# GAP-LAB-CUHK-SZ/REC-MV

Hardware: AMD Instinct MI355X
Metric: optimiser iters/sec, female-3-casual-like 512x512 (synthetic frames) (higher is better)
Workload: dtype f32

## Files before the change

rec-mv_amd/csrc/common.h:

```cpp
#pragma once
#include <hip/hip_runtime.h>
#include <stdint.h>
#include <stdio.h>
#include <string.h>
#include "../../include/recmv_hip.h"

namespace recmv {

void set_error(const char* fmt, ...);

inline int check_launch(const char* what) {
  hipError_t e = hipGetLastError();
  if (e != hipSuccess) {
    set_error("%s: %s", what, hipGetErrorString(e));
    return RECMV_ERR_HIP;
  }
  return RECMV_OK;
}

#define RECMV_HIP_TRY(expr)                                              \
  do {                                                                   \
    hipError_t e__ = (expr);                                             \
    if (e__ != hipSuccess) {                                             \
      ::recmv::set_error("%s: %s", #expr, hipGetErrorString(e__));       \
      return RECMV_ERR_HIP;                                              \
    }                                                                    \
  } while (0)

#define RECMV_REQUIRE(cond, ...)                                         \
  do {                                                                   \
    if (!(cond)) {                                                       \
      ::recmv::set_error(__VA_ARGS__);                                   \
      return RECMV_ERR_ARG;                                              \
    }                                                                    \
  } while (0)

constexpr int kWave = 64;
constexpr int kNumCU = 256;
constexpr int kNumXCD = 8;

inline int64_t ceil_div(int64_t a, int64_t b) { return (a + b - 1) / b; }

inline int stream_grid(int64_t work_items, int block) {
  int64_t g = ceil_div(work_items, block);
  const int64_t cap = (int64_t)kNumCU * 8;
  if (g > cap) g = cap;
  if (g < 1) g = 1;
  return (int)g;
}

}
```

rec-mv_amd/csrc/gemm_f32.hip:

```cpp
#include <mutex>
#include <unordered_map>
#include <type_traits>
#include <vector>
#include "common.h"
#ifdef RECMV_LIBM_SOFTPLUS
#define RECMV_EXPF(x) expf(x)
#define RECMV_LOG1PF(t) log1pf(t)
#else
#define RECMV_EXPF(x) __expf(x)
#define RECMV_LOG1PF(t) __logf(1.f + (t))
#endif

#include <algorithm>

namespace recmv {
namespace {

typedef float f32x16 __attribute__((ext_vector_type(16)));
typedef float f32x2 __attribute__((ext_vector_type(2)));
typedef __bf16 bf16x2 __attribute__((ext_vector_type(2)));
typedef __bf16 bf16x8 __attribute__((ext_vector_type(8)));
typedef unsigned int u32x4 __attribute__((ext_vector_type(4)));

struct Pieces {
  bf16x8 h, m, l;
};
__device__ __forceinline__ unsigned pack_bf16(float a, float b) {
#ifdef RECMV_SPLIT_INT
  unsigned ua = __float_as_uint(a), ub = __float_as_uint(b);
  ua += 0x7fffu + ((ua >> 16) & 1u);
  ub += 0x7fffu + ((ub >> 16) & 1u);
  return (ua >> 16) | (ub & 0xffff0000u);
#else
  const f32x2 v = {a, b};
  return __builtin_bit_cast(unsigned, __builtin_convertvector(v, bf16x2));
#endif
}
__device__ __forceinline__ void split2(float x0, float x1, unsigned& h, unsigned& m, unsigned& l) {
  h = pack_bf16(x0, x1);
  const f32x2 r = {x0 - __uint_as_float(h << 16), x1 - __uint_as_float(h & 0xffff0000u)};
  m = pack_bf16(r.x, r.y);
  const f32x2 q = {r.x - __uint_as_float(m << 16), r.y - __uint_as_float(m & 0xffff0000u)};
  l = pack_bf16(q.x, q.y);
}
__device__ __forceinline__ Pieces split8(float4 a, float4 b) {
  unsigned h[4], m[4], l[4];
  split2(a.x, a.y, h[0], m[0], l[0]);
  split2(a.z, a.w, h[1], m[1], l[1]);
  split2(b.x, b.y, h[2], m[2], l[2]);
  split2(b.z, b.w, h[3], m[3], l[3]);
  Pieces p;
  p.h = __builtin_bit_cast(bf16x8, (u32x4){h[0], h[1], h[2], h[3]});
  p.m = __builtin_bit_cast(bf16x8, (u32x4){m[0], m[1], m[2], m[3]});
  p.l = __builtin_bit_cast(bf16x8, (u32x4){l[0], l[1], l[2], l[3]});
  return p;
}

constexpr int BM = 128, BN = 128, BK = 32;
constexpr int kBlk = 256;
constexpr int LDK = BK + 4;
constexpr int LDM = BM + 4;

__device__ __forceinline__ int64_t xcd_remap(int64_t b, int64_t nb) {
  const int64_t per = nb / kNumXCD;
  if (b >= per * kNumXCD) return b;
  return (b % kNumXCD) * per + b / kNumXCD;
}

template <int ACT>
__device__ __forceinline__ float apply_act(float z, float p, float inv_p) {
  if (ACT == RECMV_ACT_RELU) return z > 0.f ? z : 0.f;
  if (ACT == RECMV_ACT_SOFTPLUS) {
    const float zb = z * p;
    const float t = RECMV_EXPF(-fabsf(zb));
    const float series = t * (1.f - t * (0.5f - t * (0.33333334f - 0.25f * t)));
    const float l = t < 0.015625f ? series : RECMV_LOG1PF(t);
    const float y = (fmaxf(zb, 0.f) + l) * inv_p;
    return zb > 20.f ? z : y;
  }
  if (ACT == RECMV_ACT_TANH) return tanhf(z);
  return z;
}

__device__ __forceinline__ float dact_y(float y, int act, float p) {
  switch (act) {
    case RECMV_ACT_RELU: return y > 0.f ? 1.f : 0.f;
    case RECMV_ACT_SOFTPLUS: {
      const float t = p * y;
      const float series = t * (1.f - t * (0.5f - t * (0.16666667f - 0.041666668f * t)));
      return t < 0.015625f ? series : 1.f - RECMV_EXPF(-t);
    }
    case RECMV_ACT_TANH: return 1.f - y * y;
    default: return 1.f;
  }
}

struct AMul {
  const float* Y;
  int64_t ldy;
  int act;
  float param, y_scale, a_scale;
  const float* B2;
  const float* bias2;
  int split;
};

__device__ __forceinline__ float4 amul4(float4 a, float4 y, const AMul& m) {
  a.x *= dact_y(y.x * m.y_scale, m.act, m.param) * m.a_scale;
  a.y *= dact_y(y.y * m.y_scale, m.act, m.param) * m.a_scale;
  a.z *= dact_y(y.z * m.y_scale, m.act, m.param) * m.a_scale;
  a.w *= dact_y(y.w * m.y_scale, m.act, m.param) * m.a_scale;
  return a;
}

__device__ __forceinline__ float4 load4_guard(const float* __restrict__ p, int64_t limit, bool vec_ok) {
  float4 v = make_float4(0.f, 0.f, 0.f, 0.f);
  if (limit >= 4 && vec_ok) {
    v = *reinterpret_cast<const float4*>(p);
  } else {
    if (limit > 0) v.x = p[0];
    if (limit > 1) v.y = p[1];
    if (limit > 2) v.z = p[2];
    if (limit > 3) v.w = p[3];
  }
  return v;
}

__device__ __forceinline__ float4 emul4(float4 v, const AMul& m, int gm, int gn, int N) {
  const float* y = m.Y + (int64_t)gm * m.ldy + gn;
  float4 yv = make_float4(0.f, 0.f, 0.f, 0.f);
  if (gn + 4 <= N && (m.ldy & 3) == 0 && (reinterpret_cast<uintptr_t>(m.Y) & 15) == 0) {
    yv = *reinterpret_cast<const float4*>(y);
  } else {
    yv.x = y[0];
    if (gn + 1 < N) yv.y = y[1];
    if (gn + 2 < N) yv.z = y[2];
    if (gn + 3 < N) yv.w = y[3];
  }
  v.x *= dact_y(yv.x * m.y_scale, m.act, m.param) * m.a_scale;
  v.y *= dact_y(yv.y * m.y_scale, m.act, m.param) * m.a_scale;
  v.z *= dact_y(yv.z * m.y_scale, m.act, m.param) * m.a_scale;
  v.w *= dact_y(yv.w * m.y_scale, m.act, m.param) * m.a_scale;
  return v;
}

template <int TBM, int TBN, int ACT>
__device__ __forceinline__ void nt_epilogue_rows(const float* __restrict__ Cs, const float* __restrict__ bias,
                                                 float* __restrict__ C, int64_t ldc, int M, int N, int m0, int n0,
                                                 float act_param, float out_scale, bool c_vec, const AMul& em) {
  constexpr int LDC = TBN + 4;
  constexpr int C4 = TBN / 4;
  constexpr int ROWS_PER_PASS = kBlk / C4;
  const int tid = threadIdx.x;
  const int c4 = tid % C4, r0 = tid / C4;
  const int gn = n0 + c4 * 4;
  if (gn >= N) return;
  const float inv_p = act_param != 0.f ? 1.f / act_param : 0.f;
  float4 bv = make_float4(0.f, 0.f, 0.f, 0.f);
  if (bias) {
    bv.x = bias[gn];
    if (gn + 1 < N) bv.y = bias[gn + 1];
    if (gn + 2 < N) bv.z = bias[gn + 2];
    if (gn + 3 < N) bv.w = bias[gn + 3];
  }
  const bool full4 = c_vec && gn + 4 <= N;
#pragma unroll 2
  for (int row = r0; row < TBM; row += ROWS_PER_PASS) {
    const int gm = m0 + row;
    if (gm >= M) break;
    float4 v = *reinterpret_cast<const float4*>(Cs + row * LDC + c4 * 4);
    v.x = apply_act<ACT>(v.x + bv.x, act_param, inv_p) * out_scale;
    v.y = apply_act<ACT>(v.y + bv.y, act_param, inv_p) * out_scale;
    v.z = apply_act<ACT>(v.z + bv.z, act_param, inv_p) * out_scale;
    v.w = apply_act<ACT>(v.w + bv.w, act_param, inv_p) * out_scale;
    if (em.Y) v = emul4(v, em, gm, gn, N);
    float* dst = C + (int64_t)gm * ldc + gn;
    if (full4) {
      *reinterpret_cast<float4*>(dst) = v;
    } else {
      dst[0] = v.x;
      if (gn + 1 < N) dst[1] = v.y;
      if (gn + 2 < N) dst[2] = v.z;
      if (gn + 3 < N) dst[3] = v.w;
    }
  }
}

template <int T, int ACT>
__device__ __forceinline__ void nt_epilogue(const float* __restrict__ Cs, const float* __restrict__ bias,
                                            float* __restrict__ C, int64_t ldc, int M, int N, int m0, int n0,
                                            float act_param, float out_scale, bool c_vec, const AMul& em) {
  nt_epilogue_rows<64 * T, 64 * T, ACT>(Cs, bias, C, ldc, M, N, m0, n0, act_param, out_scale, c_vec, em);
}

template <int T, bool FAST, bool AMUL, bool BF3>
__global__ __launch_bounds__(kBlk) void gemm_nt_kernel(const float* __restrict__ A, int64_t lda,
                                                       const float* __restrict__ B, int64_t ldb,
                                                       const float* __restrict__ bias, float* __restrict__ C,
                                                       int64_t ldc, int M, int N, int K, int act,
                                                       float act_param, float out_scale, int nbm, int nbn,
                                                       bool a_vec, bool b_vec, bool c_vec, AMul am) {
  constexpr int TBM = 64 * T, TBN = 64 * T;
  constexpr int WT = 32 * T;
  constexpr int NLD = TBM * 8 / kBlk;
  extern __shared__ __attribute__((aligned(16))) float smem[];
  float* As = smem;
  float* Bs = smem + 2 * TBM * LDK;
  const int tid = threadIdx.x, lane = tid & 63, wave = tid >> 6;
  const int wm = wave >> 1, wn = wave & 1;
  const int64_t logical = xcd_remap(blockIdx.x, (int64_t)nbm * nbn);
  const int tile_m = (int)(logical / nbn), tile_n = (int)(logical % nbn);
  const int m0 = tile_m * TBM, n0 = tile_n * TBN;
  if (am.B2 && m0 >= am.split) {
    B = am.B2;
    bias = am.bias2;
  }

  f32x16 acc[T][T];
#pragma unroll
  for (int a = 0; a < T; ++a)
#pragma unroll
    for (int b = 0; b < T; ++b)
#pragma unroll
      for (int r = 0; r < 16; ++r) acc[a][b][r] = 0.f;

// ... 895 lines not shown

  f32x16 acc[2][2];
#pragma unroll
  for (int a = 0; a < 2; ++a)
#pragma unroll
    for (int b = 0; b < 2; ++b)
#pragma unroll
      for (int r = 0; r < 16; ++r) acc[a][b][r] = 0.f;

  float4 ra[NLD], rb[NLD];
  const bool whole_mn = m0 + BM <= M && n0 + BN <= N;
  auto gload = [&](int64_t k0) {
    const bool whole = whole_mn && k0 + BKT <= kend;
#pragma unroll
    for (int r = 0; r < NLD; ++r) {
      const int idx = tid + kBlk * r;
      const int krow = idx >> 5, c4 = idx & 31;
      const int64_t k = k0 + krow;
      const int cm = m0 + c4 * 4, cn = n0 + c4 * 4;
      if (whole) {
        ra[r] = *reinterpret_cast<const float4*>(A + k * lda + cm);
        rb[r] = *reinterpret_cast<const float4*>(B + k * ldb + cn);
      } else {
        const bool kin = k < kend, ain = kin && cm < M, bin = kin && cn < N;
        const int64_t kc = kin ? k : kend - 1;
        float4 a = *reinterpret_cast<const float4*>(A + kc * lda + (cm < M ? cm : (M - 1) & ~3));
        float4 b = *reinterpret_cast<const float4*>(B + kc * ldb + (cn < N ? cn : (N - 1) & ~3));
        ra[r] = make_float4(ain ? a.x : 0.f, ain ? a.y : 0.f, ain ? a.z : 0.f, ain ? a.w : 0.f);
        rb[r] = make_float4(bin ? b.x : 0.f, bin ? b.y : 0.f, bin ? b.z : 0.f, bin ? b.w : 0.f);
      }
    }
  };
  auto lstore = [&]() {
#pragma unroll
    for (int r = 0; r < NLD; ++r) {
      const int idx = tid + kBlk * r;
      const int krow = idx >> 5, c4 = idx & 31;
      *reinterpret_cast<float4*>(As + krow * LDM + c4 * 4) = ra[r];
      *reinterpret_cast<float4*>(Bs + krow * LDM + c4 * 4) = rb[r];
    }
  };

  const int nk = (int)((kend - kbeg + BKT - 1) / BKT);
  if (nk > 0) {
    gload(kbeg);
    lstore();
  }
  __syncthreads();
  const int acol = wm * 64 + (lane & 31), bcol = wn * 64 + (lane & 31), kh = lane >> 5;
  const float* as = As + kh * LDM + acol;
  const float* bs = Bs + kh * LDM + bcol;
  for (int kt = 0; kt < nk; ++kt) {
    if (kt + 1 < nk) gload(kbeg + (int64_t)(kt + 1) * BKT);
#pragma unroll
    for (int k2 = 0; k2 < BKT / 2; ++k2) {
      const float a0 = as[k2 * 2 * LDM], a1 = as[k2 * 2 * LDM + 32];
      const float b0 = bs[k2 * 2 * LDM], b1 = bs[k2 * 2 * LDM + 32];
      acc[0][0] = __builtin_amdgcn_mfma_f32_32x32x2f32(a0, b0, acc[0][0], 0, 0, 0);
      acc[0][1] = __builtin_amdgcn_mfma_f32_32x32x2f32(a0, b1, acc[0][1], 0, 0, 0);
      acc[1][0] = __builtin_amdgcn_mfma_f32_32x32x2f32(a1, b0, acc[1][0], 0, 0, 0);
      acc[1][1] = __builtin_amdgcn_mfma_f32_32x32x2f32(a1, b1, acc[1][1], 0, 0, 0);
    }
    __syncthreads();
    if (kt + 1 < nk) lstore();
    __syncthreads();
  }

  float* Ps = P + (int64_t)split * M * N;
#pragma unroll
  for (int ni = 0; ni < 2; ++ni) {
    const int gn = n0 + wn * 64 + ni * 32 + (lane & 31);
    if (gn >= N) continue;
#pragma unroll
    for (int mi = 0; mi < 2; ++mi) {
#pragma unroll
      for (int r = 0; r < 16; ++r) {
        const int gm = m0 + wm * 64 + mi * 32 + (r & 3) + 8 * (r >> 2) + 4 * (lane >> 5);
        if (gm < M) Ps[(int64_t)gm * N + gn] = acc[mi][ni][r];
      }
    }
  }
}

__global__ __launch_bounds__(kBlk) void splitk_reduce_kernel(const float* __restrict__ P, float* __restrict__ C,
                                                             int64_t ldc, int M, int N, int splits) {
  const int64_t total = (int64_t)M * N;
  for (int64_t i = (int64_t)blockIdx.x * kBlk + threadIdx.x; i < total; i += (int64_t)gridDim.x * kBlk) {
    float s = 0.f;
    for (int sp = 0; sp < splits; ++sp) s += P[(int64_t)sp * total + i];
    C[(i / N) * ldc + (i % N)] = s;
  }
}

__global__ __launch_bounds__(kBlk) void splitk_reduce4_kernel(const float4* __restrict__ P, float* __restrict__ C,
                                                              int64_t ldc, int M, int N, int splits) {
  const int64_t total4 = (int64_t)M * N / 4;
  for (int64_t i = (int64_t)blockIdx.x * kBlk + threadIdx.x; i < total4; i += (int64_t)gridDim.x * kBlk) {
    float4 s = make_float4(0.f, 0.f, 0.f, 0.f);
    int sp = 0;
    for (; sp + 8 <= splits; sp += 8) {
      float4 v[8];
#pragma unroll
      for (int u = 0; u < 8; ++u) v[u] = P[(int64_t)(sp + u) * total4 + i];
#pragma unroll
      for (int u = 0; u < 8; ++u) {
        s.x += v[u].x;
        s.y += v[u].y;
        s.z += v[u].z;
        s.w += v[u].w;
      }
    }
    for (; sp < splits; ++sp) {
      const float4 v = P[(int64_t)sp * total4 + i];
      s.x += v.x;
      s.y += v.y;
      s.z += v.z;
      s.w += v.w;
    }
    const int64_t e = i * 4;
    *reinterpret_cast<float4*>(C + (e / N) * ldc + (e % N)) = s;
  }
}

struct PeWeights {
  float w[32];
};
__global__ __launch_bounds__(kBlk) void posenc_kernel(const float* __restrict__ x, int64_t ldx,
                                                      float* __restrict__ out, int64_t ldo, int64_t ldo_fill,
                                                      int64_t P, int L, PeWeights w, float out_scale) {
  const int nf = 1 + 2 * L;
  const int64_t total = P * nf;
  for (int64_t e = (int64_t)blockIdx.x * kBlk + threadIdx.x; e < total; e += (int64_t)gridDim.x * kBlk) {
    const int64_t p = e / nf;
    const int f = (int)(e % nf);
    const float x0 = x[p * ldx], x1 = x[p * ldx + 1], x2 = x[p * ldx + 2];
    float* o = out + p * ldo + 3 * f;
    if (f == 0) {
      o[0] = x0 * out_scale;
      o[1] = x1 * out_scale;
      o[2] = x2 * out_scale;
      for (int64_t c = 3 * nf; c < ldo_fill; ++c) out[p * ldo + c] = 0.f;
    } else {
      const int band = (f - 1) >> 1;
      const float freq = (float)(1 << band);
      const float wt = w.w[f - 1];
      float v0, v1, v2;
      if ((f - 1) & 1) {
        v0 = cosf(x0 * freq); v1 = cosf(x1 * freq); v2 = cosf(x2 * freq);
      } else {
        v0 = sinf(x0 * freq); v1 = sinf(x1 * freq); v2 = sinf(x2 * freq);
      }
      o[0] = wt * v0 * out_scale;
      o[1] = wt * v1 * out_scale;
      o[2] = wt * v2 * out_scale;
    }
  }
}

struct LaunchRec {
  hipEvent_t a, b;
  int variant;
  double flops, bytes;
};
struct Profiler {
  bool on = false;
  double min_flops = 0.0;
  double untimed[14][2] = {};
  std::vector<LaunchRec> recs;
  std::vector<hipEvent_t> pool;
  double large[14][3] = {};
  double timed_bytes[14] = {};
  double busy_union_s = 0.0, busy_span_s = 0.0;
  std::mutex mu;
  hipEvent_t get() {
    std::lock_guard<std::mutex> lk(mu);
    if (!pool.empty()) {
      hipEvent_t e = pool.back();
      pool.pop_back();
      return e;
    }
    hipEvent_t e;
    if (hipEventCreate(&e) != hipSuccess) return nullptr;
    return e;
  }
};
Profiler g_prof;

struct ScopedLaunchTimer {
  LaunchRec r;
  hipStream_t s;
  bool active;
  ScopedLaunchTimer(int variant, double M, double N, double K, hipStream_t stream) : s(stream), active(g_prof.on) {
    if (!active) return;
    const double flops = 2.0 * M * N * K;
    r.bytes = 4.0 * (M * K + N * K + M * N);
    if (flops < g_prof.min_flops) {
      std::lock_guard<std::mutex> lk(g_prof.mu);
      g_prof.untimed[variant][0] += 1.0;
      g_prof.untimed[variant][1] += flops;
      active = false;
      return;
    }
    r.variant = variant;
// ... 212 lines not shown
  }
  std::lock_guard<std::mutex> lock(g_b3_mu);
  g_b3[B] = B3Entry{(const char*)planes, N, K, ldb, Kp};
  return RECMV_OK;
}

extern "C" int recmv_b3_forget(const float* B) {
  std::lock_guard<std::mutex> lock(g_b3_mu);
  g_b3.erase(B);
  return RECMV_OK;
}

extern "C" int recmv_gemm_nt(const float* A, int64_t lda, const float* B, int64_t ldb, const float* bias,
                             float* C, int64_t ldc, int64_t M, int64_t N, int64_t K, int act,
                             float act_param, float out_scale, void* stream) {
  RECMV_REQUIRE(M >= 0 && N >= 0 && K >= 0, "gemm_nt: negative size");
  if (M == 0 || N == 0) return RECMV_OK;
  RECMV_REQUIRE(A && B && C, "gemm_nt: NULL pointer");
  RECMV_REQUIRE(lda >= K && ldb >= K && ldc >= N, "gemm_nt: leading dimension too small");
  RECMV_REQUIRE(M < (1ll << 31) - BM && N < (1ll << 31) - BN && K < (1ll << 31) - BK, "gemm_nt: size overflow");
  RECMV_REQUIRE(act >= RECMV_ACT_NONE && act <= RECMV_ACT_TANH, "gemm_nt: unknown activation %d", act);
  AMul am = {nullptr, 0, RECMV_ACT_NONE, 0.f, 1.f, 1.f};
  return dispatch_nt<false>(A, lda, B, ldb, bias, C, ldc, M, N, K, act, act_param, out_scale, am, (hipStream_t)stream);
}

extern "C" int recmv_gemm_nt_actgrad(const float* G, int64_t ldg, const float* Y, int64_t ldy, const float* B,
                                     int64_t ldb, float* C, int64_t ldc, int64_t M, int64_t N, int64_t K, int act,
                                     float act_param, float y_scale, float g_scale, void* stream) {
  RECMV_REQUIRE(M >= 0 && N >= 0 && K >= 0, "gemm_nt_actgrad: negative size");
  if (M == 0 || N == 0) return RECMV_OK;
  RECMV_REQUIRE(G && Y && B && C, "gemm_nt_actgrad: NULL pointer");
  RECMV_REQUIRE((ldg >= K || ldg == 0) && ldy >= K && ldb >= K && ldc >= N,
                "gemm_nt_actgrad: leading dimension too small");
  RECMV_REQUIRE(M < (1ll << 31) - BM && N < (1ll << 31) - BN && K < (1ll << 31) - BK, "gemm_nt_actgrad: size overflow");
  RECMV_REQUIRE(act >= RECMV_ACT_NONE && act <= RECMV_ACT_TANH, "gemm_nt_actgrad: unknown activation %d", act);
  AMul am = {Y, ldy, act, act_param, y_scale, g_scale};
  return dispatch_nt<true>(G, ldg, B, ldb, nullptr, C, ldc, M, N, K, RECMV_ACT_NONE, 0.f, 1.f, am, (hipStream_t)stream);
}

extern "C" int recmv_gemm_nt_mulgrad(const float* A, int64_t lda, const float* B, int64_t ldb, float* C, int64_t ldc,
                                     int64_t M, int64_t N, int64_t K, const float* Y, int64_t ldy, int act,
                                     float act_param, float y_scale, float scale, void* stream) {
  RECMV_REQUIRE(M >= 0 && N >= 0 && K >= 0, "gemm_nt_mulgrad: negative size");
  if (M == 0 || N == 0) return RECMV_OK;
  RECMV_REQUIRE(A && B && C && Y, "gemm_nt_mulgrad: NULL pointer");
  RECMV_REQUIRE(lda >= K && ldb >= K && ldc >= N && ldy >= N, "gemm_nt_mulgrad: leading dimension too small");
  RECMV_REQUIRE(M < (1ll << 31) - BM && N < (1ll << 31) - BN && K < (1ll << 31) - BK, "gemm_nt_mulgrad: size overflow");
  RECMV_REQUIRE(act >= RECMV_ACT_NONE && act <= RECMV_ACT_TANH, "gemm_nt_mulgrad: unknown activation %d", act);
  AMul em = {Y, ldy, act, act_param, y_scale, scale};
  return dispatch_nt<false>(A, lda, B, ldb, nullptr, C, ldc, M, N, K, RECMV_ACT_NONE, 0.f, 1.f, em, (hipStream_t)stream);
}

extern "C" int recmv_gemm_nt_seg(const float* A, int64_t lda, const float* B, int64_t ldb, const float* bias,
                                 const float* B2, const float* bias2, int64_t split_row, float* C, int64_t ldc, int64_t M,
                                 int64_t N, int64_t K, int act, float act_param, float out_scale, void* stream) {
  RECMV_REQUIRE(M >= 0 && N >= 0 && K >= 0, "gemm_nt_seg: negative size");
  if (M == 0 || N == 0) return RECMV_OK;
  RECMV_REQUIRE(A && B && C, "gemm_nt_seg: NULL pointer");
  RECMV_REQUIRE(lda >= K && ldb >= K && ldc >= N, "gemm_nt_seg: leading dimension too small");
  RECMV_REQUIRE(M < (1ll << 31) - BM && N < (1ll << 31) - BN && K < (1ll << 31) - BK, "gemm_nt_seg: size overflow");
  RECMV_REQUIRE(act >= RECMV_ACT_NONE && act <= RECMV_ACT_TANH, "gemm_nt_seg: unknown activation %d", act);
  RECMV_REQUIRE(!B2 || (split_row >= 0 && split_row % BM == 0), "gemm_nt_seg: split_row must be a multiple of %d", BM);
  RECMV_REQUIRE(!B2 || !bias == !bias2, "gemm_nt_seg: both nets with or both without a bias");
  AMul am = {nullptr, 0, RECMV_ACT_NONE, 0.f, 1.f, 1.f, B2, bias2, (int)(split_row < M ? split_row : M)};
  return dispatch_nt<false>(A, lda, B, ldb, bias, C, ldc, M, N, K, act, act_param, out_scale, am, (hipStream_t)stream);
}

extern "C" int recmv_gemm_nt_mulgrad_seg(const float* A, int64_t lda, const float* B, const float* B2, int64_t split_row,
                                         int64_t ldb, float* C, int64_t ldc, int64_t M, int64_t N, int64_t K, const float* Y,
                                         int64_t ldy, int act, float act_param, float y_scale, float scale, void* stream) {
  RECMV_REQUIRE(M >= 0 && N >= 0 && K >= 0, "gemm_nt_mulgrad_seg: negative size");
  if (M == 0 || N == 0) return RECMV_OK;
  RECMV_REQUIRE(A && B && C && Y, "gemm_nt_mulgrad_seg: NULL pointer");
  RECMV_REQUIRE(lda >= K && ldb >= K && ldc >= N && ldy >= N, "gemm_nt_mulgrad_seg: leading dimension too small");
  RECMV_REQUIRE(M < (1ll << 31) - BM && N < (1ll << 31) - BN && K < (1ll << 31) - BK, "gemm_nt_mulgrad_seg: size overflow");
  RECMV_REQUIRE(act >= RECMV_ACT_NONE && act <= RECMV_ACT_TANH, "gemm_nt_mulgrad_seg: unknown activation %d", act);
  RECMV_REQUIRE(!B2 || (split_row >= 0 && split_row % BM == 0), "gemm_nt_mulgrad_seg: split_row must be a multiple of %d", BM);
  AMul em = {Y, ldy, act, act_param, y_scale, scale, B2, nullptr, (int)(split_row < M ? split_row : M)};
  return dispatch_nt<false>(A, lda, B, ldb, nullptr, C, ldc, M, N, K, RECMV_ACT_NONE, 0.f, 1.f, em, (hipStream_t)stream);
}

extern "C" int64_t recmv_gemm_tn_workspace_bytes(int64_t M, int64_t N, int64_t K) {
  if (M <= 0 || N <= 0 || K <= 0) return 0;
  return (int64_t)tn_splits(M, N, K) * M * N * 4;
}

extern "C" int recmv_gemm_tn(const float* A, int64_t lda, const float* B, int64_t ldb, float* C, int64_t ldc,
                             int64_t M, int64_t N, int64_t K, void* workspace, int64_t workspace_bytes,
                             void* stream) {
  RECMV_REQUIRE(M >= 0 && N >= 0 && K >= 0, "gemm_tn: negative size");
  if (M == 0 || N == 0) return RECMV_OK;
  RECMV_REQUIRE(A && B && C, "gemm_tn: NULL pointer");
  RECMV_REQUIRE(lda >= M && ldb >= N && ldc >= N, "gemm_tn: leading dimension too small");
  RECMV_REQUIRE(M < (1 << 20) && N < (1 << 20), "gemm_tn: output too large");
  hipStream_t s = (hipStream_t)stream;
  if (K == 0) {
    for (int64_t m = 0; m < M; ++m) RECMV_HIP_TRY(hipMemsetAsync(C + m * ldc, 0, N * 4, s));
    return RECMV_OK;
  }
  const int splits = tn_splits(M, N, K);
  const int64_t need = (int64_t)splits * M * N * 4;
  if (!workspace || workspace_bytes < need) {
    set_error("gemm_tn: workspace %lld < %lld bytes", (long long)workspace_bytes, (long long)need);
    return RECMV_ERR_WORKSPACE;
  }
  static bool attr_set = false;
  if (!attr_set) {
    RECMV_HIP_TRY(hipFuncSetAttribute((const void*)gemm_tn_kernel<false>, hipFuncAttributeMaxDynamicSharedMemorySize,
                                      kTnLds));
    RECMV_HIP_TRY(hipFuncSetAttribute((const void*)gemm_tn_kernel<true>, hipFuncAttributeMaxDynamicSharedMemorySize,
                                      kTnLds));
    attr_set = true;
  }
  const int nbm = (int)ceil_div(M, BM), nbn = (int)ceil_div(N, BN);
  int64_t kchunk = ceil_div(ceil_div(K, splits), BK) * BK;
  const bool a_vec = aligned16(A) && lda % 4 == 0, b_vec = aligned16(B) && ldb % 4 == 0;
  int rc;
  {
  ScopedLaunchTimer timer(8, (double)M, (double)N, (double)K, s);
  const bool bf3_tn = g_gemm_mode == 1 && (g_b3_families & 4);
  if (!bf3_tn && tn_occ() && a_vec && b_vec && lda >= ((M + 3) & ~3ll) && ldb >= ((N + 3) & ~3ll) && M >= 4 && N >= 4) {
    kchunk = ceil_div(ceil_div(K, splits), 16) * 16;
    hipLaunchKernelGGL(gemm_tn_occ_kernel<16>, dim3((unsigned)(nbm * nbn * splits)), dim3(kBlk), 2 * 16 * LDM * 4, s, A, lda,
                       B, ldb, (float*)workspace, (int)M, (int)N, K, nbm, nbn, kchunk);
  } else if (bf3_tn)
    hipLaunchKernelGGL(gemm_tn_kernel<true>, dim3((unsigned)(nbm * nbn * splits)), dim3(kBlk), kTnLds, s, A, lda, B,
                       ldb, (float*)workspace, (int)M, (int)N, K, nbm, nbn, kchunk, a_vec, b_vec);
  else
    hipLaunchKernelGGL(gemm_tn_kernel<false>, dim3((unsigned)(nbm * nbn * splits)), dim3(kBlk), kTnLds, s, A, lda, B,
                       ldb, (float*)workspace, (int)M, (int)N, K, nbm, nbn, kchunk, a_vec, b_vec);
  rc = check_launch("gemm_tn");
  }
  if (rc) return rc;
  if (N % 4 == 0 && ldc % 4 == 0 && aligned16(C) && aligned16(workspace))
    hipLaunchKernelGGL(splitk_reduce4_kernel, dim3(stream_grid(M * N / 4, kBlk)), dim3(kBlk), 0, s,
                       (const float4*)workspace, C, ldc, (int)M, (int)N, splits);
  else
    hipLaunchKernelGGL(splitk_reduce_kernel, dim3(stream_grid(M * N, kBlk)), dim3(kBlk), 0, s,
                       (const float*)workspace, C, ldc, (int)M, (int)N, splits);
  return check_launch("gemm_tn/reduce");
}

extern "C" int recmv_posenc_forward(const float* x, int64_t ldx, float* out, int64_t ldo, int64_t ldo_fill,
                                    int64_t P, int L, const float* weights_host, float out_scale,
                                    void* stream) {
  RECMV_REQUIRE(P >= 0 && L >= 0 && L <= 16, "posenc: bad size (P=%lld, L=%d)", (long long)P, L);
  if (P == 0) return RECMV_OK;
  RECMV_REQUIRE(x && out, "posenc: NULL pointer");
  RECMV_REQUIRE(ldx >= 3 && ldo >= 3 + 6 * L && ldo_fill <= ldo, "posenc: leading dimension too small");
  hipStream_t s = (hipStream_t)stream;
  PeWeights hw;
  for (int i = 0; i < 32; ++i) hw.w[i] = (weights_host && i < 2 * L) ? weights_host[i] : 1.f;
  hipLaunchKernelGGL(posenc_kernel, dim3(stream_grid(P * (1 + 2 * L), kBlk)), dim3(kBlk), 0, s, x, ldx, out, ldo,
                     ldo_fill, P, L, hw, out_scale);
  return check_launch("posenc");
}

extern "C" int recmv_profile_begin(double min_flops) {
  g_prof.recs.clear();
  for (auto& u : g_prof.untimed) u[0] = u[1] = 0.0;
  g_prof.min_flops = min_flops;
  g_prof.on = true;
  return RECMV_OK;
}

extern "C" int recmv_profile_bytes(double* out, int n_variants) {
  RECMV_REQUIRE(out && n_variants >= 9, "profile_bytes: need room for 9 variants");
  for (int i = 0; i < n_variants; ++i) out[i] = 0.0;
  auto slot = [&](int v) { return v < n_variants ? v : (v == 11 ? 7 : (v == 12 ? 2 : (v == 13 ? 6 : 3))); };
  for (int v = 0; v < 14; ++v) out[slot(v)] += g_prof.timed_bytes[v];
  return RECMV_OK;
}

extern "C" int recmv_profile_large(double* out, int n_variants) {
  RECMV_REQUIRE(out && n_variants >= 9, "profile_large: need room for 9 variants");
  for (int i = 0; i < 3 * n_variants; ++i) out[i] = 0.0;
  auto slot = [&](int v) { return v < n_variants ? v : (v == 11 ? 7 : (v == 12 ? 2 : (v == 13 ? 6 : 3))); };
  for (int v = 0; v < 14; ++v)
    for (int q = 0; q < 3; ++q) out[3 * slot(v) + q] += g_prof.large[v][q];
  return RECMV_OK;
}

extern "C" int recmv_profile_busy(double* out2) {
  RECMV_REQUIRE(out2, "profile_busy: NULL");
  out2[0] = g_prof.busy_union_s;
  out2[1] = g_prof.busy_span_s;
  return RECMV_OK;
}

extern "C" int recmv_profile_end(double* out, int n_variants) {
  g_prof.on = false;
  RECMV_REQUIRE(out && n_variants >= 9, "profile_end: need room for 9 variants");
  for (int i = 0; i < 5 * n_variants; ++i) out[i] = 0.0;
  auto slot = [&](int v) { return v < n_variants ? v : (v == 11 ? 7 : (v == 12 ? 2 : (v == 13 ? 6 : 3))); };
  for (int v = 0; v < 14; ++v) {
    out[5 * slot(v) + 3] += g_prof.untimed[v][0];
    out[5 * slot(v) + 4] += g_prof.untimed[v][1];
  }
  std::vector<std::pair<double, double>> iv;
  iv.reserve(g_prof.recs.size());
  hipEvent_t origin = g_prof.recs.empty() ? nullptr : g_prof.recs.front().a;
  for (auto& b : g_prof.timed_bytes) b = 0.0;
  for (auto& l : g_prof.large) l[0] = l[1] = l[2] = 0.0;
  for (auto& r : g_prof.recs) {
    g_prof.timed_bytes[r.variant] += r.bytes;
    RECMV_HIP_TRY(hipEventSynchronize(r.b));
    float ms = 0.f;
    RECMV_HIP_TRY(hipEventElapsedTime(&ms, r.a, r.b));
    if (r.flops >= 4.0e9) {
      g_prof.large[r.variant][0] += 1.0;
      g_prof.large[r.variant][1] += (double)ms * 1e-3;
      g_prof.large[r.variant][2] += r.flops;
    }
    out[5 * slot(r.variant) + 0] += 1.0;
    out[5 * slot(r.variant) + 1] += (double)ms * 1e-3;
    out[5 * slot(r.variant) + 2] += r.flops;
    float t0 = 0.f;
    if (r.a != origin && hipEventElapsedTime(&t0, origin, r.a) != hipSuccess) t0 = -1.f;
    if (t0 >= 0.f) iv.emplace_back((double)t0 * 1e-3, (double)(t0 + ms) * 1e-3);
  }
  for (auto& r : g_prof.recs) {
    g_prof.pool.push_back(r.a);
    g_prof.pool.push_back(r.b);
  }
  g_prof.recs.clear();
// ... 20 lines not shown
```

rec-mv_amd/csrc/linear_bwd.hip:

```cpp
#include "common.h"

namespace recmv {
namespace {

constexpr int kBlk = 256;
constexpr int kColTile = 64;
constexpr int kMaxChunks = 96;

__global__ __launch_bounds__(kBlk) void colsum_partial_kernel(const float* __restrict__ g, int64_t ld, int64_t rows,
                                                              int cols, int64_t rows_per_chunk,
                                                              float* __restrict__ partial) {
  __shared__ float sh[kBlk / kColTile][kColTile];
  const int ctile = blockIdx.x, chunk = blockIdx.y;
  const int lane = threadIdx.x % kColTile, rgrp = threadIdx.x / kColTile;
  const int c = ctile * kColTile + lane;
  const int64_t r0 = (int64_t)chunk * rows_per_chunk;
  int64_t r1 = r0 + rows_per_chunk;
  if (r1 > rows) r1 = rows;
  float s = 0.f;
  if (c < cols)
    for (int64_t r = r0 + rgrp; r < r1; r += kBlk / kColTile) s += g[r * ld + c];
  sh[rgrp][lane] = s;
  __syncthreads();
  if (rgrp == 0 && c < cols) {
    float t = 0.f;
#pragma unroll
    for (int q = 0; q < kBlk / kColTile; ++q) t += sh[q][lane];
    partial[(int64_t)chunk * cols + c] = t;
  }
}

__device__ __forceinline__ float dact_y(float y, int act, float p) {
  switch (act) {
    case RECMV_ACT_RELU: return y > 0.f ? 1.f : 0.f;
    case RECMV_ACT_SOFTPLUS: return -expm1f(-p * y);
    case RECMV_ACT_TANH: return 1.f - y * y;
    default: return 1.f;
  }
}

template <int VEC>
__global__ __launch_bounds__(kBlk) void act_grad_colsum_kernel(const float* __restrict__ gy, int64_t ldg,
                                                               const float* __restrict__ y, int64_t ldy,
                                                               float* __restrict__ gz, int64_t ldz, int64_t rows,
                                                               int cols, int64_t rows_per_chunk, int act, float p,
                                                               float* __restrict__ partial) {
  constexpr int CT = kColTile / VEC;
  constexpr int RG = kBlk / CT;
  __shared__ float sh[RG][kColTile];
  const int ctile = blockIdx.x, chunk = blockIdx.y;
  const int cl = threadIdx.x % CT, rgrp = threadIdx.x / CT;
  const int c = ctile * kColTile + cl * VEC;
  const int64_t r0 = (int64_t)chunk * rows_per_chunk;
  int64_t r1 = r0 + rows_per_chunk;
  if (r1 > rows) r1 = rows;
  float s[VEC];
#pragma unroll
  for (int v = 0; v < VEC; ++v) s[v] = 0.f;
  if (c < cols) {
    for (int64_t r = r0 + rgrp; r < r1; r += RG) {
      if (VEC == 4) {
        const float4 g4 = *reinterpret_cast<const float4*>(gy + r * ldg + c);
        const float4 y4 = *reinterpret_cast<const float4*>(y + r * ldy + c);
        float4 o;
        o.x = g4.x * dact_y(y4.x, act, p);
        o.y = g4.y * dact_y(y4.y, act, p);
        o.z = g4.z * dact_y(y4.z, act, p);
        o.w = g4.w * dact_y(y4.w, act, p);
        *reinterpret_cast<float4*>(gz + r * ldz + c) = o;
        s[0] += o.x;
        s[VEC > 1 ? 1 : 0] += o.y;
        s[VEC > 2 ? 2 : 0] += o.z;
        s[VEC > 3 ? 3 : 0] += o.w;
      } else {
        const float v = gy[r * ldg + c] * dact_y(y[r * ldy + c], act, p);
        gz[r * ldz + c] = v;
        s[0] += v;
      }
    }
  }
#pragma unroll
  for (int v = 0; v < VEC; ++v) sh[rgrp][cl * VEC + v] = s[v];
  __syncthreads();
  if (threadIdx.x < kColTile) {
    const int cc = ctile * kColTile + threadIdx.x;
    if (cc < cols) {
      float t = 0.f;
#pragma unroll
      for (int q = 0; q < RG; ++q) t += sh[q][threadIdx.x];
      partial[(int64_t)chunk * cols + cc] = t;
    }
  }
}

__global__ __launch_bounds__(kBlk) void colsum_final_kernel(const float* __restrict__ partial, int chunks, int cols,
                                                            float* __restrict__ out) {
  const int c = blockIdx.x * kBlk + threadIdx.x;
  if (c >= cols) return;
  float s = 0.f;
  int q = 0;
  for (; q + 8 <= chunks; q += 8) {
    float v[8];
#pragma unroll
    for (int u = 0; u < 8; ++u) v[u] = partial[(int64_t)(q + u) * cols + c];
#pragma unroll
    for (int u = 0; u < 8; ++u) s += v[u];
  }
  for (; q < chunks; ++q) s += partial[(int64_t)q * cols + c];
  out[c] = s;
}

inline int colsum_chunks(int64_t rows) {
  int64_t ch = ceil_div(rows, 256);
  if (ch > kMaxChunks) ch = kMaxChunks;
  if (ch < 1) ch = 1;
  return (int)ch;
}

inline int64_t align256(int64_t b) { return (b + 255) / 256 * 256; }

}
}

using namespace recmv;

extern "C" int64_t recmv_colsum_workspace_bytes(int64_t rows, int64_t cols) {
  if (rows <= 0 || cols <= 0) return 0;
  return (int64_t)colsum_chunks(rows) * cols * 4;
}

extern "C" int recmv_colsum(const float* g, int64_t ld, int64_t rows, int64_t cols, float* out, void* workspace,
                            int64_t workspace_bytes, void* stream) {
  RECMV_REQUIRE(rows >= 0 && cols >= 0 && cols < (1 << 24), "colsum: bad size");
  if (cols == 0) return RECMV_OK;
  RECMV_REQUIRE(out, "colsum: NULL output");
  hipStream_t s = (hipStream_t)stream;
  if (rows == 0) {
    RECMV_HIP_TRY(hipMemsetAsync(out, 0, cols * 4, s));
    return RECMV_OK;
  }
  RECMV_REQUIRE(g && ld >= cols, "colsum: bad input");
  const int chunks = colsum_chunks(rows);
  if (!workspace || workspace_bytes < (int64_t)chunks * cols * 4) {
    set_error("colsum: workspace too small");
    return RECMV_ERR_WORKSPACE;
  }
  const int64_t rpc = ceil_div(rows, chunks);
  hipLaunchKernelGGL(colsum_partial_kernel, dim3((unsigned)ceil_div(cols, kColTile), (unsigned)chunks), dim3(kBlk), 0, s,
                     g, ld, rows, (int)cols, rpc, (float*)workspace);
  int rc = check_launch("colsum/partial");
  if (rc) return rc;
  hipLaunchKernelGGL(colsum_final_kernel, dim3((unsigned)ceil_div(cols, kBlk)), dim3(kBlk), 0, s,
                     (const float*)workspace, chunks, (int)cols, out);
  return check_launch("colsum/final");
}

extern "C" int64_t recmv_linear_backward_workspace_bytes(int64_t M, int64_t N, int64_t K) {
  if (M <= 0 || N <= 0) return 256;
  return align256(M * ((N + 3) & ~3ll) * 4) + align256(recmv_gemm_tn_workspace_bytes(N, K, M)) +
         align256(recmv_colsum_workspace_bytes(M, N)) + 256;
}

extern "C" int recmv_linear_backward(const float* gy, int64_t ldgy, const float* y, int64_t ldy, const float* x,
                                     int64_t ldx, const float* Wt, int64_t ldwt, int64_t M, int64_t N, int64_t K,
                                     int act, float act_param, float* gx, int64_t ldgx, float* gW, float* gb,
                                     void* workspace, int64_t workspace_bytes, void* stream) {
  RECMV_REQUIRE(M >= 0 && N >= 0 && K >= 0, "linear_backward: negative size");
  RECMV_REQUIRE(gy && (act == RECMV_ACT_NONE || y), "linear_backward: NULL pointer");
  const int64_t need = recmv_linear_backward_workspace_bytes(M, N, K);
  if (!workspace || workspace_bytes < need) {
    set_error("linear_backward: workspace %lld < %lld bytes", (long long)workspace_bytes, (long long)need);
    return RECMV_ERR_WORKSPACE;
  }
  char* ws = (char*)workspace;
  float* gzbuf = (float*)ws;
  const int64_t ldz = (N + 3) & ~3ll;
  char* tn_ws = ws + align256(M * ldz * 4);
  const int64_t tn_bytes = align256(recmv_gemm_tn_workspace_bytes(N, K, M));
  char* cs_ws = tn_ws + tn_bytes;
  const int64_t cs_bytes = align256(recmv_colsum_workspace_bytes(M, N));
  const float* gz = gy;
  int64_t ldgz = ldgy;
  int rc;
  bool gb_done = false;
  if (act != RECMV_ACT_NONE && M > 0 && N > 0) {
    if (gb) {
      const int chunks = colsum_chunks(M);
      const int64_t rpc = ceil_div(M, chunks);
      const bool vec = N % 4 == 0 && ldgy % 4 == 0 && ldy % 4 == 0 &&
                       ((reinterpret_cast<uintptr_t>(gy) | reinterpret_cast<uintptr_t>(y)) & 15) == 0;
      if (vec)
        hipLaunchKernelGGL(act_grad_colsum_kernel<4>, dim3((unsigned)ceil_div(N, kColTile), (unsigned)chunks), dim3(kBlk),
                           0, (hipStream_t)stream, gy, ldgy, y, ldy, gzbuf, ldz, M, (int)N, rpc, act, act_param,
                           (float*)cs_ws);
      else
        hipLaunchKernelGGL(act_grad_colsum_kernel<1>, dim3((unsigned)ceil_div(N, kColTile), (unsigned)chunks), dim3(kBlk),
                           0, (hipStream_t)stream, gy, ldgy, y, ldy, gzbuf, ldz, M, (int)N, rpc, act, act_param,
                           (float*)cs_ws);
      rc = check_launch("linear_backward/act_grad_colsum");
      if (rc) return rc;
      hipLaunchKernelGGL(colsum_final_kernel, dim3((unsigned)ceil_div(N, kBlk)), dim3(kBlk), 0, (hipStream_t)stream,
                         (const float*)cs_ws, chunks, (int)N, gb);
      rc = check_launch("linear_backward/colsum_final");
      if (rc) return rc;
      gb_done = true;
    } else {
      rc = recmv_act_grad_2d(gy, ldgy, y, ldy, gzbuf, ldz, M, N, act, act_param, 1.f, 1.f, stream);
      if (rc) return rc;
    }
    gz = gzbuf;
    ldgz = ldz;
  }
  if (gb && !gb_done) {
    rc = recmv_colsum(gz, ldgz, M, N, gb, cs_ws, cs_bytes, stream);
    if (rc) return rc;
  }
  if (gx && K > 0) {
    RECMV_REQUIRE(Wt, "linear_backward: gx needs W^T");
    rc = recmv_gemm_nt(gz, ldgz, Wt, ldwt, nullptr, gx, ldgx, M, K, N, RECMV_ACT_NONE, 0.f, 1.f, stream);
    if (rc) return rc;
  }
  if (gW && K > 0) {
    RECMV_REQUIRE(x, "linear_backward: gW needs x");
    rc = recmv_gemm_tn(gz, ldgz, x, ldx, gW, K, N, K, M, tn_ws, tn_bytes, stream);
    if (rc) return rc;
  }
  return RECMV_OK;
}
```

Measured before the change: 10.05.

## Fuse activation-gradient and bias colsum into split-K weight-gradient GEMM

```diff
diff --git a/rec-mv_amd/csrc/common.h b/rec-mv_amd/csrc/common.h
--- a/rec-mv_amd/csrc/common.h
+++ b/rec-mv_amd/csrc/common.h
@@ -49,4 +49,25 @@
   return (int)g;
 }
 
+#ifdef __HIPCC__
+__device__ __forceinline__ float dact_y(float y, int act, float p) {
+  switch (act) {
+    case RECMV_ACT_RELU: return y > 0.f ? 1.f : 0.f;
+    case RECMV_ACT_SOFTPLUS: return -expm1f(-p * y);
+    case RECMV_ACT_TANH: return 1.f - y * y;
+    default: return 1.f;
+  }
 }
+#endif
+
+
+bool linear_bwd_fused();
+
+int gemm_tn_actgrad_colsum(const float* A, int64_t lda, const float* B, int64_t ldb, float* C, int64_t ldc, int64_t M,
+                           int64_t N, int64_t K, void* workspace, int64_t workspace_bytes, void* stream, const float* Y,
+                           int64_t ldy, int act, float act_param, float* gb, int64_t colsum_rows, bool* taken);
+
+int gemm_nt_actgrad_exact(const float* G, int64_t ldg, const float* Y, int64_t ldy, const float* B, int64_t ldb, float* C,
+                          int64_t ldc, int64_t M, int64_t N, int64_t K, int act, float act_param, void* stream);
+
+}
diff --git a/rec-mv_amd/csrc/gemm_f32.hip b/rec-mv_amd/csrc/gemm_f32.hip
--- a/rec-mv_amd/csrc/gemm_f32.hip
+++ b/rec-mv_amd/csrc/gemm_f32.hip
@@ -82,8 +82,11 @@
   return z;
 }
 
-__device__ __forceinline__ float dact_y(float y, int act, float p) {
+constexpr int kActSoftplusLibm = 0x10 | RECMV_ACT_SOFTPLUS;
+
+__device__ __forceinline__ float dact_y_hw(float y, int act, float p) {
   switch (act) {
+    case kActSoftplusLibm: return dact_y(y, RECMV_ACT_SOFTPLUS, p);
     case RECMV_ACT_RELU: return y > 0.f ? 1.f : 0.f;
     case RECMV_ACT_SOFTPLUS: {
       const float t = p * y;
@@ -106,10 +109,10 @@
 };
 
 __device__ __forceinline__ float4 amul4(float4 a, float4 y, const AMul& m) {
-  a.x *= dact_y(y.x * m.y_scale, m.act, m.param) * m.a_scale;
-  a.y *= dact_y(y.y * m.y_scale, m.act, m.param) * m.a_scale;
-  a.z *= dact_y(y.z * m.y_scale, m.act, m.param) * m.a_scale;
-  a.w *= dact_y(y.w * m.y_scale, m.act, m.param) * m.a_scale;
+  a.x *= dact_y_hw(y.x * m.y_scale, m.act, m.param) * m.a_scale;
+  a.y *= dact_y_hw(y.y * m.y_scale, m.act, m.param) * m.a_scale;
+  a.z *= dact_y_hw(y.z * m.y_scale, m.act, m.param) * m.a_scale;
+  a.w *= dact_y_hw(y.w * m.y_scale, m.act, m.param) * m.a_scale;
   return a;
 }
 
@@ -137,10 +140,10 @@
     if (gn + 2 < N) yv.z = y[2];
     if (gn + 3 < N) yv.w = y[3];
   }
-  v.x *= dact_y(yv.x * m.y_scale, m.act, m.param) * m.a_scale;
-  v.y *= dact_y(yv.y * m.y_scale, m.act, m.param) * m.a_scale;
-  v.z *= dact_y(yv.z * m.y_scale, m.act, m.param) * m.a_scale;
-  v.w *= dact_y(yv.w * m.y_scale, m.act, m.param) * m.a_scale;
+  v.x *= dact_y_hw(yv.x * m.y_scale, m.act, m.param) * m.a_scale;
+  v.y *= dact_y_hw(yv.y * m.y_scale, m.act, m.param) * m.a_scale;
+  v.z *= dact_y_hw(yv.z * m.y_scale, m.act, m.param) * m.a_scale;
+  v.w *= dact_y_hw(yv.w * m.y_scale, m.act, m.param) * m.a_scale;
   return v;
 }
 
@@ -1202,6 +1205,174 @@
   }
 }
 
+template <int BKT, int ACT>
+__global__ __launch_bounds__(kBlk, 4) void gemm_tn_occ_dz_kernel(const float* __restrict__ A, int64_t lda,
+                                                                 const float* __restrict__ B, int64_t ldb,
+                                                                 const float* __restrict__ Y, int64_t ldy,
+                                                                 float act_param, float* __restrict__ P,
+                                                                 float* __restrict__ colpart, int M, int N, int64_t K,
+                                                                 int nbm, int nbn, int64_t kchunk, int64_t colsum_rows) {
+  constexpr int NLD = BKT * 32 / kBlk;
+  extern __shared__ __attribute__((aligned(16))) float smem[];
+  float* As = smem;
+  float* Bs = smem + BKT * LDM;
+  const int tid = threadIdx.x, lane = tid & 63, wave = tid >> 6;
+  const int wm = wave >> 1, wn = wave & 1;
+  const int tiles = nbm * nbn;
+  int split = blockIdx.x / tiles, tile = blockIdx.x % tiles;
+  const int splits = gridDim.x / tiles;
+  if (splits % kNumXCD == 0) {
+    const int x = blockIdx.x % kNumXCD, j = blockIdx.x / kNumXCD;
+    split = x + kNumXCD * (j / tiles);
+    tile = j % tiles;
+  }
+  const int tile_m = tile / nbn, tile_n = tile % nbn;
+  const int m0 = tile_m * BM, n0 = tile_n * BN;
+  const int64_t kbeg = (int64_t)split * kchunk;
+  int64_t kend = kbeg + kchunk;
+  if (kend > K) kend = K;
+  const bool do_cs = colpart != nullptr && tile_n == 0;
+
+  f32x16 acc[2][2];
+#pragma unroll
+  for (int a = 0; a < 2; ++a)
+#pragma unroll
+    for (int b = 0; b < 2; ++b)
+#pragma unroll
+      for (int r = 0; r < 16; ++r) acc[a][b][r] = 0.f;
+
+  float4 ra[NLD], rb[NLD], ry[NLD];
+  float4* csl = reinterpret_cast<float4*>(smem + 2 * BKT * LDM) + tid;
+  if (do_cs) *csl = make_float4(0.f, 0.f, 0.f, 0.f);
+  int kst = 0;
+  const int cs_rows = (int)(colsum_rows - kbeg < 0 ? 0 : (colsum_rows - kbeg < kchunk ? colsum_rows - kbeg : kchunk));
+  const int krows = (int)(kend - kbeg);
+  constexpr bool HASY = ACT != RECMV_ACT_NONE;
+  auto dz4 = [&](float4 a, float4 y) {
+    a.x *= dact_y(y.x, ACT, act_param);
+    a.y *= dact_y(y.y, ACT, act_param);
+    a.z *= dact_y(y.z, ACT, act_param);
+    a.w *= dact_y(y.w, ACT, act_param);
+    return a;
+  };
+  unsigned offa[NLD], offb[NLD], offy[NLD];
+#pragma unroll
+  for (int r = 0; r < NLD; ++r) {
+    const int idx = tid + kBlk * r;
+    const int krow = idx >> 5, c4 = idx & 31;
+    offa[r] = (unsigned)(krow * (int)lda + m0 + c4 * 4);
+    offb[r] = (unsigned)(krow * (int)ldb + n0 + c4 * 4);
+    offy[r] = HASY ? (unsigned)(krow * (int)ldy + m0 + c4 * 4) : 0u;
+  }
+  auto gload = [&](int kt0) {
+    kst = kt0;
+    const float* Ak = A + (kbeg + kt0) * lda;
+    const float* Bk = B + (kbeg + kt0) * ldb;
+    const bool whole = kt0 + BKT <= krows;
+#pragma unroll
+    for (int r = 0; r < NLD; ++r) {
+      const int krow = (tid + kBlk * r) >> 5;
+      if (whole || kt0 + krow < krows) {
+        ra[r] = *reinterpret_cast<const float4*>(Ak + offa[r]);
+        rb[r] = *reinterpret_cast<const float4*>(Bk + offb[r]);
+      } else {
+        ra[r] = make_float4(0.f, 0.f, 0.f, 0.f);
+        rb[r] = make_float4(0.f, 0.f, 0.f, 0.f);
+      }
+    }
+  };
+  auto yload = [&]() {
+    if (!HASY) return;
+    const float* Yk = Y + (kbeg + kst) * ldy;
+    const bool whole = kst + BKT <= krows;
+#pragma unroll
+    for (int r = 0; r < NLD; ++r) {
+      const int krow = (tid + kBlk * r) >> 5;
+      if (whole || kst + krow < krows)
+        ry[r] = *reinterpret_cast<const float4*>(Yk + offy[r]);
+      else
+        ry[r] = make_float4(0.f, 0.f, 0.f, 0.f);
+    }
+  };
+  auto lstore = [&]() {
+#pragma unroll
+    for (int r = 0; r < NLD; ++r) {
+      const int idx = tid + kBlk * r;
+      const int krow = idx >> 5, c4 = idx & 31;
+      if (HASY) ra[r] = dz4(ra[r], ry[r]);
+      *reinterpret_cast<float4*>(As + krow * LDM + c4 * 4) = ra[r];
+      *reinterpret_cast<float4*>(Bs + krow * LDM + c4 * 4) = rb[r];
+    }
+    if (do_cs) {
+      float4 cs = *csl;
+#pragma unroll
+      for (int r = 0; r < NLD; ++r) {
+        if (kst + ((tid + kBlk * r) >> 5) < cs_rows) {
+          cs.x += ra[r].x;
+          cs.y += ra[r].y;
+          cs.z += ra[r].z;
+          cs.w += ra[r].w;
+        }
+      }
+      *csl = cs;
+    }
+  };
+
+  const int nk = (int)((kend - kbeg + BKT - 1) / BKT);
+  if (nk > 0) {
+    gload(0);
+    yload();
+    lstore();
+  }
+  __syncthreads();
+  const int acol = wm * 64 + (lane & 31), bcol = wn * 64 + (lane & 31), kh = lane >> 5;
+  const float* as = As + kh * LDM + acol;
+  const float* bs = Bs + kh * LDM + bcol;
+  for (int kt = 0; kt < nk; ++kt) {
+    if (kt + 1 < nk) gload((kt + 1) * BKT);
+#pragma unroll
+    for (int k2 = 0; k2 < BKT / 2; ++k2) {
+      const float a0 = as[k2 * 2 * LDM], a1 = as[k2 * 2 * LDM + 32];
+      const float b0 = bs[k2 * 2 * LDM], b1 = bs[k2 * 2 * LDM + 32];
+      acc[0][0] = __builtin_amdgcn_mfma_f32_32x32x2f32(a0, b0, acc[0][0], 0, 0, 0);
+      acc[0][1] = __builtin_amdgcn_mfma_f32_32x32x2f32(a0, b1, acc[0][1], 0, 0, 0);
+      acc[1][0] = __builtin_amdgcn_mfma_f32_32x32x2f32(a1, b0, acc[1][0], 0, 0, 0);
+      acc[1][1] = __builtin_amdgcn_mfma_f32_32x32x2f32(a1, b1, acc[1][1], 0, 0, 0);
+    }
+    if (kt + 1 < nk) yload();
+    __syncthreads();
+    if (kt + 1 < nk) lstore();
+    __syncthreads();
+  }
+
+  float* Ps = P + (int64_t)split * M * N;
+#pragma unroll
+  for (int ni = 0; ni < 2; ++ni) {
+    const int gn = n0 + wn * 64 + ni * 32 + (lane & 31);
+    if (gn >= N) continue;
+#pragma unroll
+    for (int mi = 0; mi < 2; ++mi) {
+#pragma unroll
+      for (int r = 0; r < 16; ++r) {
+        const int gm = m0 + wm * 64 + mi * 32 + (r & 3) + 8 * (r >> 2) + 4 * (lane >> 5);
+        if (gm < M) Ps[(int64_t)gm * N + gn] = acc[mi][ni][r];
+      }
+    }
+  }
+
+  if (do_cs) {
+    float* red = smem;
+    *reinterpret_cast<float4*>(red + (tid >> 5) * BM + (tid & 31) * 4) = *csl;
+    __syncthreads();
+    if (tid < BM && m0 + tid < M) {
+      float v = 0.f;
+#pragma unroll
+      for (int q = 0; q < kBlk / 32; ++q) v += red[q * BM + tid];
+      colpart[(int64_t)split * M + m0 + tid] = v;
+    }
+  }
+}
+
 __global__ __launch_bounds__(kBlk) void splitk_reduce_kernel(const float* __restrict__ P, float* __restrict__ C,
                                                              int64_t ldc, int M, int N, int splits) {
   const int64_t total = (int64_t)M * N;
@@ -1239,6 +1410,53 @@
     }
     const int64_t e = i * 4;
     *reinterpret_cast<float4*>(C + (e / N) * ldc + (e % N)) = s;
+  }
+}
+
+__global__ __launch_bounds__(kBlk) void splitk_reduce4_colsum_kernel(const float4* __restrict__ P, float* __restrict__ C,
+                                                                     int64_t ldc, int M, int N, int splits,
+                                                                     const float* __restrict__ colpart,
+                                                                     float* __restrict__ gb) {
+  const int64_t total4 = (int64_t)M * N / 4;
+  for (int64_t i = (int64_t)blockIdx.x * kBlk + threadIdx.x; i < total4; i += (int64_t)gridDim.x * kBlk) {
+    float4 s = make_float4(0.f, 0.f, 0.f, 0.f);
+    int sp = 0;
+    for (; sp + 8 <= splits; sp += 8) {
+      float4 v[8];
+#pragma unroll
+      for (int u = 0; u < 8; ++u) v[u] = P[(int64_t)(sp + u) * total4 + i];
+#pragma unroll
+      for (int u = 0; u < 8; ++u) {
+        s.x += v[u].x;
+        s.y += v[u].y;
+        s.z += v[u].z;
+        s.w += v[u].w;
+      }
+    }
+    for (; sp < splits; ++sp) {
+      const float4 v = P[(int64_t)sp * total4 + i];
+      s.x += v.x;
+      s.y += v.y;
+      s.z += v.z;
+      s.w += v.w;
+    }
+    const int64_t e = i * 4;
+    *reinterpret_cast<float4*>(C + (e / N) * ldc + (e % N)) = s;
+  }
+  if (gb) {
+    for (int64_t m = (int64_t)blockIdx.x * kBlk + threadIdx.x; m < M; m += (int64_t)gridDim.x * kBlk) {
+      float s = 0.f;
+      int sp = 0;
+      for (; sp + 8 <= splits; sp += 8) {
+        float v[8];
+#pragma unroll
+        for (int u = 0; u < 8; ++u) v[u] = colpart[(int64_t)(sp + u) * M + m];
+#pragma unroll
+        for (int u = 0; u < 8; ++u) s += v[u];
+      }
+      for (; sp < splits; ++sp) s += colpart[(int64_t)sp * M + m];
+      gb[m] = s;
+    }
   }
 }
 
@@ -1617,7 +1835,7 @@
 
 extern "C" int64_t recmv_gemm_tn_workspace_bytes(int64_t M, int64_t N, int64_t K) {
   if (M <= 0 || N <= 0 || K <= 0) return 0;
-  return (int64_t)tn_splits(M, N, K) * M * N * 4;
+  return (int64_t)tn_splits(M, N, K) * (M * N + M) * 4;
 }
 
 extern "C" int recmv_gemm_tn(const float* A, int64_t lda, const float* B, int64_t ldb, float* C, int64_t ldc,
@@ -1676,6 +1894,73 @@
   return check_launch("gemm_tn/reduce");
 }
 
+namespace recmv {
+
+bool linear_bwd_fused() {
+  static const bool v = [] { const char* e = getenv("RECMV_LINEAR_BWD_FUSED"); return !(e && e[0] == '0'); }();
+  return v;
+}
+
+int gemm_tn_actgrad_colsum(const float* A, int64_t lda, const float* B, int64_t ldb, float* C, int64_t ldc, int64_t M,
+                           int64_t N, int64_t K, void* workspace, int64_t workspace_bytes, void* stream, const float* Y,
+                           int64_t ldy, int act, float act_param, float* gb, int64_t colsum_rows, bool* taken) {
+  *taken = false;
+  if (!linear_bwd_fused() || M <= 0 || N <= 0 || K <= 0 || !A || !B || !C) return RECMV_OK;
+  if (act < RECMV_ACT_NONE || act > RECMV_ACT_TANH || (act != RECMV_ACT_NONE && !Y)) return RECMV_OK;
+  if (act == RECMV_ACT_NONE) Y = nullptr;
+  if (!Y && !gb) return RECMV_OK;
+  if (lda < M || ldb < N || ldc < N || (Y && ldy < M) || M >= (1 << 20) || N >= (1 << 20)) return RECMV_OK;
+  if (lda >= (1 << 26) || ldb >= (1 << 26) || ldy >= (1 << 26)) return RECMV_OK;
+  const bool bf3_tn = g_gemm_mode == 1 && (g_b3_families & 4);
+  const bool ok = !bf3_tn && tn_occ() && aligned16(A) && lda % 4 == 0 && aligned16(B) && ldb % 4 == 0 && M % BM == 0 &&
+                  N % BN == 0 && (!Y || (aligned16(Y) && ldy % 4 == 0)) && ldc % 4 == 0 && aligned16(C) &&
+                  aligned16(workspace);
+  if (!ok) return RECMV_OK;
+  const int splits = tn_splits(M, N, K);
+  const int64_t part_bytes = (int64_t)splits * M * N * 4;
+  if (!workspace || workspace_bytes < part_bytes + (int64_t)splits * M * 4) return RECMV_OK;
+  if (colsum_rows > K) colsum_rows = K;
+  hipStream_t s = (hipStream_t)stream;
+  float* colpart = gb ? (float*)((char*)workspace + part_bytes) : nullptr;
+  const int nbm = (int)ceil_div(M, BM), nbn = (int)ceil_div(N, BN);
+  const int64_t kchunk = ceil_div(ceil_div(K, splits), 16) * 16;
+  int rc;
+  {
+    ScopedLaunchTimer timer(8, (double)M, (double)N, (double)K, s);
+#define RECMV_TN_DZ(ACT)                                                                                              \
+  hipLaunchKernelGGL((gemm_tn_occ_dz_kernel<16, ACT>), dim3((unsigned)(nbm * nbn * splits)), dim3(kBlk),                      \
+                     2 * 16 * LDM * 4 + kBlk * 16, s, A, lda, B, ldb, Y, ldy, act_param, (float*)workspace, colpart, (int)M, (int)N, K, nbm, nbn, kchunk,  \
+                     colsum_rows)
+    switch (act) {
+      case RECMV_ACT_RELU: RECMV_TN_DZ(RECMV_ACT_RELU); break;
+      case RECMV_ACT_SOFTPLUS: RECMV_TN_DZ(RECMV_ACT_SOFTPLUS); break;
+      case RECMV_ACT_TANH: RECMV_TN_DZ(RECMV_ACT_TANH); break;
+      default: RECMV_TN_DZ(RECMV_ACT_NONE); break;
+    }
+#undef RECMV_TN_DZ
+    rc = check_launch("gemm_tn(dz)");
+  }
+  if (rc) return rc;
+  hipLaunchKernelGGL(splitk_reduce4_colsum_kernel, dim3(stream_grid(M * N / 4, kBlk)), dim3(kBlk), 0, s,
+                     (const float4*)workspace, C, ldc, (int)M, (int)N, splits, (const float*)colpart, gb);
+  rc = check_launch("gemm_tn(dz)/reduce");
+  if (rc) return rc;
+  *taken = true;
+  return RECMV_OK;
+}
+
+int gemm_nt_actgrad_exact(const float* G, int64_t ldg, const float* Y, int64_t ldy, const float* B, int64_t ldb, float* C,
+                          int64_t ldc, int64_t M, int64_t N, int64_t K, int act, float act_param, void* stream) {
+  if (M == 0 || N == 0) return RECMV_OK;
+  RECMV_REQUIRE(G && Y && B && C, "gemm_nt_actgrad: NULL pointer");
+  RECMV_REQUIRE(ldg >= K && ldy >= K && ldb >= K && ldc >= N, "gemm_nt_actgrad: leading dimension too small");
+  RECMV_REQUIRE(M < (1ll << 31) - BM && N < (1ll << 31) - BN && K < (1ll << 31) - BK, "gemm_nt_actgrad: size overflow");
+  AMul am = {Y, ldy, act == RECMV_ACT_SOFTPLUS ? kActSoftplusLibm : act, act_param, 1.f, 1.f};
+  return dispatch_nt<true>(G, ldg, B, ldb, nullptr, C, ldc, M, N, K, RECMV_ACT_NONE, 0.f, 1.f, am, (hipStream_t)stream);
+}
+
+}
+
 extern "C" int recmv_posenc_forward(const float* x, int64_t ldx, float* out, int64_t ldo, int64_t ldo_fill,
                                     int64_t P, int L, const float* weights_host, float out_scale,
                                     void* stream) {
diff --git a/rec-mv_amd/csrc/linear_bwd.hip b/rec-mv_amd/csrc/linear_bwd.hip
--- a/rec-mv_amd/csrc/linear_bwd.hip
+++ b/rec-mv_amd/csrc/linear_bwd.hip
@@ -27,15 +27,6 @@
 #pragma unroll
     for (int q = 0; q < kBlk / kColTile; ++q) t += sh[q][lane];
     partial[(int64_t)chunk * cols + c] = t;
-  }
-}
-
-__device__ __forceinline__ float dact_y(float y, int act, float p) {
-  switch (act) {
-    case RECMV_ACT_RELU: return y > 0.f ? 1.f : 0.f;
-    case RECMV_ACT_SOFTPLUS: return -expm1f(-p * y);
-    case RECMV_ACT_TANH: return 1.f - y * y;
-    default: return 1.f;
   }
 }
 
@@ -183,6 +174,22 @@
   int64_t ldgz = ldgy;
   int rc;
   bool gb_done = false;
+  if (gW && x && M > 0 && N > 0 && K > 0 && (gb || act != RECMV_ACT_NONE)) {
+    bool taken = false;
+    rc = gemm_tn_actgrad_colsum(gy, ldgy, x, ldx, gW, K, N, K, M, tn_ws, tn_bytes, stream, y, ldy, act, act_param, gb, M, &taken);
+    if (rc) return rc;
+    if (taken) {
+      if (gx) {
+        RECMV_REQUIRE(Wt, "linear_backward: gx needs W^T");
+        if (act != RECMV_ACT_NONE)
+          rc = gemm_nt_actgrad_exact(gy, ldgy, y, ldy, Wt, ldwt, gx, ldgx, M, K, N, act, act_param, stream);
+        else
+          rc = recmv_gemm_nt(gy, ldgy, Wt, ldwt, nullptr, gx, ldgx, M, K, N, RECMV_ACT_NONE, 0.f, 1.f, stream);
+        if (rc) return rc;
+      }
+      return RECMV_OK;
+    }
+  }
   if (act != RECMV_ACT_NONE && M > 0 && N > 0) {
     if (gb) {
       const int chunks = colsum_chunks(M);
```

Measured after the change: 9.827. 0.978x the previous value.
